# lunarlab-gatech/SLIDE_SLAM

Hardware: AMD Instinct MI355X
Metric: pose-graph updates/sec + ms/Gauss-Newton iter, 8-robot 10k-landmark graph (higher is better)
Workload: dtype f64

## Files before the change

### slide_slam_amd/csrc/chol_kernels.hip

```cpp
#include <hip/hip_runtime.h>
#include <stdlib.h>
#include <algorithm>
#include <type_traits>
#include <utility>
#include <vector>

#include "graph_dev.hpp"
#include "kernels.hpp"

namespace sl {

typedef double v4d __attribute__((ext_vector_type(4)));
constexpr int CHOL_BATCH_MAX = 8;
__device__ inline v4d mfma_f64(double a, double b, v4d c) { return __builtin_amdgcn_mfma_f64_16x16x4f64(a, b, c, 0, 0, 0); }

__device__ inline double rsqrt_nr(double d) {
#ifdef SLIDE_RSQRT_OLD
  double y = __builtin_amdgcn_rsq(d);
  y = y * (1.5 - 0.5 * d * y * y);
  y = y * (1.5 - 0.5 * d * y * y);
  return y;
#else
  double y = __builtin_amdgcn_rsq(d);
  double t = d * y, h = 0.5 * y;
// ... 1736 lines not shown
}

struct ExtractArgs { int n; const double* S[CHOL_STEP_BATCH_MAX]; int ld[CHOL_STEP_BATCH_MAX]; int T[CHOL_STEP_BATCH_MAX]; int Tr[CHOL_STEP_BATCH_MAX]; double* yv[CHOL_STEP_BATCH_MAX]; double* dp[CHOL_STEP_BATCH_MAX]; int* status[CHOL_STEP_BATCH_MAX]; };
__global__ void k_chol_extract_y_b(ExtractArgs A) {
  const int r = blockIdx.y;
  const int c = blockIdx.x * blockDim.x + threadIdx.x;
  if (c == 0) A.status[r][4] = 0;
  if (c < A.T[r] * NB) {
    A.yv[r][c] = A.S[r][(size_t)c * A.ld[r] + (size_t)A.Tr[r] * NB];
    A.dp[r][c] = __longlong_as_double((long long)BWD_SENT);
  }
}

constexpr int CHAIN_THREADS = 320;
struct alignas(16) ChainLds {
  alignas(16) double xs[2][NB];
  alignas(16) double ys[NB];
  alignas(16) double red[4][NB];
  alignas(16) double Lo[6][256];
  alignas(16) double Ws[4][256];
  alignas(16) double tmp[3][256];
  alignas(16) double Ms[NB][NB + 1];
};
template <bool F32, bool WFIRE = false>
__device__ __forceinline__ void bwd_chain_body(ChainLds& W, const double* __restrict__ S, int ld, int T, const double* __restrict__ Ld,
                                               const double* __restrict__ Winv, const double* __restrict__ yv, double* dp, int* status, int bidx,
                                               const float* __restrict__ L32, const int* __restrict__ prof,
                                               const double* __restrict__ wf_prev = nullptr, double wf_thr = 0.0, int wf_Tprev = 0,
                                               int* wf_lds = nullptr, int wf_lim = 0) {
  int dummy_state = 0;
  int& wf_state = WFIRE ? *wf_lds : dummy_state;
  auto& Ms = W.Ms; auto& Lo = W.Lo; auto& Ws = W.Ws; auto& tmp = W.tmp; auto& xs = W.xs; auto& ys = W.ys;
  const int tid = threadIdx.x;
  const bool worker = tid < 256;
  CSTAMP(0);
  const int c = T - 1 - bidx;
  if (WFIRE) {
    if (tid == 0) wf_state = 0;
    __syncthreads();
  }
  const int col = tid >> 2, part = tid & 3;
  const int jtop = prof ? prof[c] : T - 1;
  const int nj = jtop - c;
  constexpr int RB = F32 ? 6 : 3;
  typedef typename std::conditional<F32, float, double>::type tile_t;
  tile_t tr[RB][16];
  const double* tcol = S + (size_t)(c * NB + col) * ld + 16 * part;
  const float* pcol = F32 ? L32 + ((size_t)c * (T - 1) - (size_t)c * (c - 1) / 2) * (NB * NB) + col * NB + 16 * part : nullptr;
  auto tile_load = [&](tile_t (&dst)[16], int q) {
    if (F32) {
      const float4* tp = reinterpret_cast<const float4*>(pcol + (size_t)(nj - 1 - q) * (NB * NB));
#pragma unroll
// ... 4 lines not shown
    } else {
      const double* tp = tcol + (size_t)(jtop - q) * NB;
#pragma unroll
      for (int r = 0; r < 16; ++r) dst[r] = tp[r];
    }
  };
  double y0 = 0.0;
  if (worker) {
#pragma unroll
    for (int q = 0; q < RB; ++q)
      if (q < nj) tile_load(tr[q], q);
    y0 = yv[c * NB + col];
  }
  if (worker) {
    const double* Ldk = Ld + (size_t)c * NB * NB;
    const double* Wk = Winv + (size_t)c * 1024;
#pragma unroll
    for (int b = 1; b < 4; ++b)
#pragma unroll
      for (int a = 0; a < b; ++a) Lo[b * (b - 1) / 2 + a][tid] = Ldk[(size_t)(16 * a + (tid >> 4)) * NB + 16 * b + (tid & 15)];
#pragma unroll
    for (int b = 0; b < 4; ++b) Ws[b][tid] = Wk[(size_t)b * 256 + tid];
  }
  __syncthreads();
  {
    const int r = tid & 15, cc = (tid >> 4) & 15;
    if (worker) {
#pragma unroll
      for (int b = 0; b < 4; ++b) Ms[16 * b + r][16 * b + cc] = Ws[b][cc * 16 + r];
    }
    __syncthreads();
#pragma unroll
    for (int d = 1; d < 4; ++d) {
#pragma unroll
      for (int a = 0; a + d < 4; ++a) {
        const int b = a + d;
        double t = 0.0;
#pragma unroll
        for (int m = a; m < b; ++m)
#pragma unroll
          for (int n = 0; n < 16; ++n) t += Lo[b * (b - 1) / 2 + m][n * 16 + r] * Ms[16 * m + n][16 * a + cc];
        if (worker) tmp[a][cc * 16 + r] = t;
      }
      __syncthreads();
#pragma unroll
      for (int a = 0; a + d < 4; ++a) {
        const int b = a + d;
// ... 60 lines not shown
        }
      }
    }
  }
  CSTAMP(4);
  if (WFIRE && wf_state != 0) {
    if (tid < NB) __hip_atomic_store(dp + (size_t)c * NB + tid, wf_prev[(size_t)c * NB + tid], __ATOMIC_RELAXED, __HIP_MEMORY_SCOPE_AGENT);
    if (tid == 0) {
      if (wf_state == 2) atomicMax(status + 7, c);
      atomicAdd(status + 3, 1);
    }
    return;
  }
  acc += __shfl_xor(acc, 1);
  acc += __shfl_xor(acc, 2);
  if (worker && part == 0) ys[col] = y0 - acc;
  __syncthreads();
  CSTAMP(5);
  double x = 0.0;
#pragma unroll
  for (int r = 0; r < 16; ++r) x += mreg[r] * ys[16 * part + r];
  x += __shfl_xor(x, 1);
  x += __shfl_xor(x, 2);
  if (worker && part == 0) __hip_atomic_store(dp + (size_t)c * NB + col, x, __ATOMIC_RELAXED, __HIP_MEMORY_SCOPE_AGENT);
  CSTAMP(6);
}
__device__ __forceinline__ int bwd_ticket(int* ctr) {
  __shared__ int s_t;
  if (threadIdx.x == 0) s_t = atomicAdd(ctr, 1);
  __syncthreads();
  const int t = s_t;
  __syncthreads();
  return t;
}
__global__ __launch_bounds__(CHAIN_THREADS) void k_chol_bwd_chain(const double* __restrict__ S, int ld, int T, const double* __restrict__ Ld,
                                                        const double* __restrict__ Winv, const double* __restrict__ yv, double* dp, int* status,
                                                        const int* __restrict__ prof) {
  __shared__ ChainLds W;
  const int t = bwd_ticket(&status[4]);
  if (t >= T) return;
  bwd_chain_body<false>(W, S, ld, T, Ld, Winv, yv, dp, status, t, nullptr, prof);
}
__global__ __launch_bounds__(CHAIN_THREADS) void k_chol_bwd_chain_wf(const double* __restrict__ S, int ld, int T, const double* __restrict__ Ld,
                                                           const double* __restrict__ Winv, const double* __restrict__ yv, double* dp, int* status,
                                                           const int* __restrict__ prof, const double* __restrict__ prev, double thr, int Tprev, int lim) {
  __shared__ ChainLds W;
  __shared__ int s_wf;
  const int t = bwd_ticket(&status[4]);
  if (t >= T) return;
  bwd_chain_body<false, true>(W, S, ld, T, Ld, Winv, yv, dp, status, t, nullptr, prof, prev, thr, Tprev, &s_wf, lim);
}
constexpr int BWD_BATCH_MAX = 32;
struct BwdBatchArgs {
  int n;
  const double* S[BWD_BATCH_MAX]; int ld[BWD_BATCH_MAX]; int T[BWD_BATCH_MAX];
  const double* Ld[BWD_BATCH_MAX]; const double* Winv[BWD_BATCH_MAX]; const double* yv[BWD_BATCH_MAX]; double* dp[BWD_BATCH_MAX];
  int* status[BWD_BATCH_MAX];
  const int* prof[BWD_BATCH_MAX];
  int base[BWD_BATCH_MAX + 1];
  int Tmax;
};
__global__ __launch_bounds__(CHAIN_THREADS) void k_chol_bwd_chain_batched(BwdBatchArgs A) {
  __shared__ ChainLds W;
  for (;;) {
    const int t = bwd_ticket(&A.status[0][4]);
    if (t >= A.n * A.Tmax) return;
    const int r = t % A.n, b = t / A.n;
    if (b >= A.T[r]) continue;
    bwd_chain_body<false>(W, A.S[r], A.ld[r], A.T[r], A.Ld[r], A.Winv[r], A.yv[r], A.dp[r], A.status[r], b, nullptr, A.prof[r]);
    return;
  }
}


enum { TAB_MF = 0, TAB_MB = 1, TAB_PF = 2, TAB_PB = 3 };
struct ChainTabArgs {
  int n; int T[CHOL_BATCH_MAX]; const double* S[CHOL_BATCH_MAX]; int ld[CHOL_BATCH_MAX];
  const double* Ld[CHOL_BATCH_MAX]; const double* Winv[CHOL_BATCH_MAX]; const int* prof[CHOL_BATCH_MAX]; double* ctab[CHOL_BATCH_MAX];
};
__global__ __launch_bounds__(256) void k_chain_tables(ChainTabArgs A) {
  __shared__ ChainLds W;
  __shared__ double Ts[NB][NB];
  auto& Ms = W.Ms; auto& Lo = W.Lo; auto& Ws = W.Ws; auto& tmp = W.tmp;
  const int sys = blockIdx.y, c = blockIdx.x, tid = threadIdx.x;
  const int T = A.T[sys];
  if (c >= T) return;
  {
    const double* Ldk = A.Ld[sys] + (size_t)c * NB * NB;
    const double* Wk = A.Winv[sys] + (size_t)c * 1024;
#pragma unroll
    for (int b = 1; b < 4; ++b)
#pragma unroll
// ... 599 lines not shown
      acc += w[t * NB + lane] * x[t * NB + lane];
    }
  } else {
    for (int q = lane; q < nrow; q += 64) acc += w[q] * x[q];
  }
#pragma unroll
  for (int m = 32; m >= 1; m >>= 1) acc += __shfl_xor(acc, m);
  if (lane == 0) A.yv[r][col] -= acc;
}
void launch_border_apply(const CholSystem* d, int n, const double* const* xloc, hipStream_t s) {
  BorderApplyArgs A{};
  A.n = n;
  int Tmax = 0;
  for (int i = 0; i < n; ++i) {
    A.S[i] = d[i].S; A.ld[i] = d[i].ld; A.T[i] = d[i].T; A.nbr[i] = d[i].nbr; A.yv[i] = d[i].yv; A.x[i] = xloc[i];
    A.b0[i] = d[i].b0 > 0 ? d[i].b0 : d[i].T;
    A.segtab[i] = d[i].segtab;
    Tmax = d[i].T > Tmax ? d[i].T : Tmax;
  }
  if (Tmax > 0) hipLaunchKernelGGL(k_border_apply, dim3(Tmax * NB / 4, 1, n), dim3(256), 0, s, A);
}

void launch_chol_bwd_all(const double* S, int ld, int T, const double* Ld, const double* Winv, double* yv, double* dp,
                         int* status, const int* prof, hipStream_t s, const double* wf_prev, double wf_thr, int wf_Tprev, int wf_lim);
void launch_chol_extract_y(const double* S, int ld, int T, double* yv, double* dp, int* status, hipStream_t s, int nbr, int b0, double* prev) {
  hipLaunchKernelGGL(k_chol_extract_y, dim3((T * NB + 255) / 256), dim3(256), 0, s, S, ld, T, (b0 > 0 ? b0 : T) + nbr, yv, dp, status, prev);
}
struct StepPlan { int kb, nP, g0, g1, nX, TvA, TvB, TvX, nbA, nbB, nbX; long long nA, nB; };
static int chol_n_cu() {
  static int n_cu = 0;
  if (!n_cu) {
    int dev = 0;
    hipDeviceProp_t pr;
    if (hipGetDevice(&dev) == hipSuccess && hipGetDeviceProperties(&pr, dev) == hipSuccess) n_cu = pr.multiProcessorCount;
    if (n_cu <= 0) n_cu = 256;
  }
  return n_cu;
}
static StepPlan plan_step(int k, int T, const int* prof, int nbr = 0, const int* bfirst = nullptr, int kofs = 0) {
  static const double frac = getenv("SLIDE_CHOL_FRAC") ? atof(getenv("SLIDE_CHOL_FRAC")) : 0.5;
  StepPlan p{};
  p.kb = k & ~1;
  p.TvA = p.TvB = p.TvX = T;
  if (prof && k < T) {
    p.TvA = prof[k] + 1;
    if (p.kb >= 1) p.TvB = prof[p.kb - 1] + 1;
    if (k >= 1) p.TvX = prof[k - 1] + 1;
// ... 185 lines not shown
  if (!solve) {
    ExtractArgs E{};
    E.n = n;
    for (int i = 0; i < n; ++i) {
      E.S[i] = d[i].S; E.ld[i] = d[i].ld; E.T[i] = d[i].T; E.Tr[i] = (d[i].b0 > 0 ? d[i].b0 : d[i].T) + d[i].nbr;
      E.yv[i] = d[i].yv; E.dp[i] = d[i].dp; E.status[i] = d[i].status;
    }
    if (Tmax > 0) hipLaunchKernelGGL(k_chol_extract_y_b, dim3((Tmax * NB + 255) / 256, n), dim3(256), 0, s, E);
    return;
  }
  launch_chain_tables(d, n, s);
  const double* yin[CHOL_BATCH_MAX];
  double* xout[CHOL_BATCH_MAX];
  for (int i = 0; i < n; ++i) {
    launch_chol_extract_y(d[i].S, d[i].ld, d[i].T, d[i].yv, d[i].dp, d[i].status, s, d[i].nbr);
    yin[i] = d[i].yv; xout[i] = d[i].dp;
  }
  if (chain_has_tables(d, n)) {
    launch_chain_batch(d, n, yin, xout, false, false, true, nullptr, s);
    return;
  }
  launch_chol_bwd_batch(d, n, s);
}
void launch_chol_bwd_batch(const CholSystem* d, int n, hipStream_t s) {
  if (n > BWD_BATCH_MAX) {
    for (int lo = 0; lo < n; lo += BWD_BATCH_MAX) launch_chol_bwd_batch(d + lo, n - lo < BWD_BATCH_MAX ? n - lo : BWD_BATCH_MAX, s);
    return;
  }
  BwdBatchArgs B{};
  B.n = n;
  B.base[0] = 0;
  int Tmax = 0;
  for (int i = 0; i < n; ++i) {
    B.S[i] = d[i].S; B.ld[i] = d[i].ld; B.T[i] = d[i].T; B.Ld[i] = d[i].Ld; B.Winv[i] = d[i].Winv; B.yv[i] = d[i].yv; B.dp[i] = d[i].dp;
    B.status[i] = d[i].status;
    B.prof[i] = d[i].prof;
    B.base[i + 1] = B.base[i] + d[i].T;
    Tmax = d[i].T > Tmax ? d[i].T : Tmax;
  }
  B.Tmax = Tmax;
  if (B.base[n] <= 0) return;
  hipLaunchKernelGGL(k_chol_bwd_chain_batched, dim3(B.base[n]), dim3(CHAIN_THREADS), 0, s, B);
}
void launch_chol_solve_bwd(const CholSystem& cs, hipStream_t s) {
  if (chain_has_tables(&cs, 1)) {
    launch_chain_tables(&cs, 1, s);
    const double* yin = cs.yv;
    double* xout = cs.dp;
    launch_chain_batch(&cs, 1, &yin, &xout, false, false, true, nullptr, s);
    return;
  }
  launch_chol_bwd_all(cs.S, cs.ld, cs.T, cs.Ld, cs.Winv, cs.yv, cs.dp, cs.status, cs.prof, s);
}
void launch_chol_bwd_all(const double* S, int ld, int T, const double* Ld, const double* Winv, double* yv, double* dp,
                         int* status, const int* prof, hipStream_t s, const double* wf_prev, double wf_thr, int wf_Tprev, int wf_lim) {
  if (wf_lim < 0 || wf_lim > wf_Tprev) wf_lim = wf_Tprev;
  if (wf_prev && wf_thr > 0.0 && wf_Tprev > 0 && wf_lim > 0)
    hipLaunchKernelGGL(k_chol_bwd_chain_wf, dim3(T), dim3(CHAIN_THREADS), 0, s, S, ld, T, Ld, Winv, yv, dp, status, prof, wf_prev, wf_thr, wf_Tprev, wf_lim);
  else
    hipLaunchKernelGGL(k_chol_bwd_chain, dim3(T), dim3(CHAIN_THREADS), 0, s, S, ld, T, Ld, Winv, yv, dp, status, prof);
}

struct CholLLPlan {
  LLSys* d_sys = nullptr; LLTask* d_tasks = nullptr; int* d_ints = nullptr;
  int n_sys = 0, n_tasks = 0, n_ints = 0, n_chain = 0, max_cols = 0;
};
CholLLPlan* chol_ll_plan_create(const CholSystem* d, int n, const int* const* h_ord, hipStream_t up) {
  static const int ll_mode = getenv("SLIDE_LL_MODE") ? atoi(getenv("SLIDE_LL_MODE")) : 0;
  std::vector<LLSys> sys(n);
  std::vector<std::vector<int>> first(n), bf(n), bphys(n), profv(n);
  size_t n_ints = 16;
  int Tmax = 0;
  for (int i = 0; i < n; ++i) {
    const CholSystem& c = d[i];
    LLSys& y = sys[i];
    y.S = c.S; y.Ld = c.Ld; y.Winv = c.Winv; y.status = c.status; y.ld = c.ld; y.T = c.T; y.B0 = c.b0 > 0 ? c.b0 : c.T; y.nbr = c.nbr;
    y.frows = y.B0 + y.nbr + 1;
    y.flags = reinterpret_cast<int*>(n_ints);
    n_ints += (size_t)y.T * y.frows;
    Tmax = c.T > Tmax ? c.T : Tmax;
    profv[i].resize(c.T);
    for (int k = 0; k < c.T; ++k) profv[i][k] = c.h_prof ? std::min(c.h_prof[k], c.T - 1) : c.T - 1;
    first[i].assign(c.T, 0);
// ... 138 lines not shown
```

### slide_slam_amd/csrc/host_graph.hip

```cpp
#include <chrono>

#include "host_graph.hpp"

#include <algorithm>
#include <cmath>
#include <cstdio>
#include <cstdlib>
#include <map>
#include <unordered_map>

namespace sl {

static inline int lam_ks_cap(int nl) {
  const int tiles = (nl + 1) * nl;
  if (tiles <= 0) return 1;
  return tiles <= 32 ? 16 : std::max(1, std::min(16, 256 / tiles));
}

thread_local std::string g_last_error;
void thread_capture_mode_local() {
  thread_local bool done = false;
  if (done) return;
  hipStreamCaptureMode m = hipStreamCaptureModeThreadLocal;
  (void)hipThreadExchangeStreamCaptureMode(&m);
// ... 532 lines not shown
    SL_HIP(hipStreamSynchronize(master));
  }
  if (!d_pair_tickets && chol_pair_mask() != 0) {
    SL_HIP(hipMalloc(reinterpret_cast<void**>(&d_pair_tickets), 12 * CHOL_STEP_BATCH_MAX * sizeof(int)));
    SL_HIP(hipMemsetAsync(d_pair_tickets, 0, 12 * CHOL_STEP_BATCH_MAX * sizeof(int), master));
    SL_HIP(hipStreamSynchronize(master));
  }
  if (!d_Gs) SL_HIP(hipMalloc(reinterpret_cast<void**>(&d_Gs), CHOL_BATCH_HOST_MAX * sizeof(GraphDev)));
  if (!d_status_all) SL_HIP(hipMalloc(reinterpret_cast<void**>(&d_status_all), CHOL_BATCH_HOST_MAX * 8 * sizeof(int)));
  SL_HIP(hipMemcpyAsync(d_Gs, hG.data(), n * sizeof(GraphDev), hipMemcpyHostToDevice, master));
  if (rb.on()) {
    hR.resize(n);
    for (int i = 0; i < n; ++i) hR[i] = member_view(graphs[i]);
    if (!d_Rs) SL_HIP(hipMalloc(reinterpret_cast<void**>(&d_Rs), CHOL_BATCH_HOST_MAX * sizeof(RobustDev)));
    SL_HIP(hipMemcpyAsync(d_Rs, hR.data(), n * sizeof(RobustDev), hipMemcpyHostToDevice, master));
  }
  if (ol.on()) {
    hO.resize(n);
    for (int i = 0; i < n; ++i) hO[i] = member_obs_view(graphs[i]);
    if (!d_Os) SL_HIP(hipMalloc(reinterpret_cast<void**>(&d_Os), CHOL_BATCH_HOST_MAX * sizeof(ObsLossDev)));
    SL_HIP(hipMemcpyAsync(d_Os, hO.data(), n * sizeof(ObsLossDev), hipMemcpyHostToDevice, master));
  }
  SL_HIP(hipStreamSynchronize(master));
  seg_sys.clear(); l2_sys.clear(); l2_graph.clear(); seg_hord.clear();
  free_ll_band_plans();
  if (arrow && hG[0].n_slots > 0) {
    for (int i = 0; i < n; ++i) {
      HostGraph* g = graphs[i];
      const GraphDev& G = hG[i];
      if (G.nsep <= 0 || g->segs.empty()) { seg_sys.push_back(sys[i]); seg_hord.push_back(nullptr); continue; }
      for (size_t k = 0; k < g->segs.size(); ++k) {
        const HostGraph::Seg sg = g->segs[k];
        CholSystem c = sys[i];
        c.S = G.S + (size_t)sg.t0 * NB * G.ld + (size_t)sg.t0 * NB;
        c.T = sg.t1 - sg.t0;
        c.Ld = G.Ld + (size_t)sg.t0 * NB * NB; c.Winv = G.Winv + (size_t)sg.t0 * 1024;
        c.yv = G.yv + (size_t)sg.t0 * NB; c.dp = G.dp + (size_t)sg.t0 * NB;
        c.h_prof = g->seg_prof[k].data(); c.prof = g->d_seg_prof.d + g->seg_prof_off[k]; c.first = nullptr;
        c.b0 = G.T - sg.t0; c.kofs = sg.t0;
        c.L32 = nullptr; c.ctab = nullptr;
        const int* hord = nullptr;
        if (k < g->seg_ord.size() && !getenv("SLIDE_SEG_PLAIN")) {
          c.h_bfirst = g->seg_sfirst[k].data();
          c.ord = g->d_seg_ord.d + k * (size_t)G.nbr;
          hord = g->seg_ord[k].data();
        }
        seg_sys.push_back(c);
        seg_hord.push_back(hord);
      }
      if (!g->seg_tab.empty() && !getenv("SLIDE_SEG_PLAIN")) sys[i].segtab = g->d_seg_tab.d;
      CholSystem l2{};
      l2.S = G.bord; l2.ld = G.ldb; l2.T = G.nsep; l2.Ld = g->d_Ld2.d; l2.Winv = g->d_Winv2.d; l2.yv = g->d_yv2.d; l2.dp = g->d_dp2.d;
      l2.status = G.status; l2.nbr = G.nbr - G.nsep;
      l2.bord = G.bord + (size_t)G.nsep * NB * G.ldb + (size_t)G.nsep * NB; l2.ldb = G.ldb;
      l2_sys.push_back(l2);
      l2_graph.push_back(i);
    }
    {
      std::vector<std::pair<int, int>> jl;
      for (int i = 0; i < n; ++i) {
        const int nb = sys[i].nbr, T = sys[i].T;
        const int* hb = sys[i].h_bfirst;
        if (nb > 1023 || n > 2047) { jl.clear(); break; }
        const std::vector<int>& stb = graphs[i]->seg_tab;
        const bool seg = sys[i].segtab != nullptr && !stb.empty();
        for (int jb = 0; jb < nb; ++jb)
          for (int ib = jb; ib <= nb; ++ib) {
            int K = T - (hb ? std::max(hb[ib], hb[jb]) : 0);
            if (seg) {
              K = 0;
              const int NS = stb[0];
// ... 492 lines not shown
      if (e1) (void)hipEventRecord(e1, master);
    } else {
      const int rc = factor_all(e1);
      if (rc != SLIDE_OK) return rc;
    }
    mark(1);
    if (n_syrk_jobs > 0) launch_border_syrk_jobs(sys.data(), n, d_syrk_jobs, n_syrk_jobs, syrk_lds_pad, master);
    else launch_border_syrk(sys.data(), n, master);
    mark(6);
    if (!l2_sys.empty()) {
      if (ll_l2) launch_chol_ll(ll_l2, l2_sys.data(), (int)l2_sys.size(), master);
      else launch_chol_batch(l2_sys.data(), (int)l2_sys.size(), d_ctr2, master, nullptr, false, 100, (chol_pair_mask() & 2) ? pair_tickets(8) : nullptr);
      if (n_l2_jobs > 0) launch_border_syrk_jobs(l2_sys.data(), (int)l2_sys.size(), d_l2_jobs, n_l2_jobs, 0, master);
      else launch_border_syrk(l2_sys.data(), (int)l2_sys.size(), master);
    }
    mark(2);
    static const bool env_canon = !(getenv("SLIDE_SEP_CANONICAL") && getenv("SLIDE_SEP_CANONICAL")[0] == '0');
    const bool canon = whole && sep_dissected() && env_canon && n <= 8;
    if (canon) launch_sep_gather(hG.data(), n, maps, Y, false, master, d_sep_tmask, sTL * NB, sep_mask_b, sep_top2, sep_ld2, sep_bord2);
    else launch_sep_gather(hG.data(), n, maps, Y, !whole, master, d_sep_tmask);
    mark(3);
  }
  if (whole || part == 2) {
    if (!whole && !owned) launch_sep_unpack(Y, master);
    if (owned) launch_sep_unpack(Y, master, sTL, sep_Ts + sep_nl);
    if (sep_dissected()) {
      const int TL = sTL, Tt = sTt;
      static const bool env_canon2 = !(getenv("SLIDE_SEP_CANONICAL") && getenv("SLIDE_SEP_CANONICAL")[0] == '0');
      const bool canon2 = whole && env_canon2 && n <= 8;
      if (!owned) {
        if (ll_leaves) launch_chol_ll(ll_leaves, lv, 2, master);
        else launch_chol_batch(lv, 2, sep_ctr2, master, nullptr, false, 100, (chol_pair_mask() & 4) ? pair_tickets(9) : nullptr);
        if (canon2) {
          CholSystem tp2[2] = {top, top};
          for (int hh = 0; hh < 2; ++hh) {
            tp2[hh].S = sepS + (size_t)(hh ? sTa : 0) * NB * ld_s; tp2[hh].T = sep_leafT[hh]; tp2[hh].b0 = sTL;
            if (hh) { tp2[hh].bord = sep_top2; tp2[hh].ldb = sep_ld2; }
          }
          CholSystem sl2[2];
          int ks_lam[2] = {1, 1};
          for (int hh = 0; hh < 2 && sep_nl > 0; ++hh) {
            CholSystem sl{};
            sl.S = sepS + (size_t)(hh ? sTa : 0) * NB * ld_s; sl.ld = ld_s; sl.T = sep_leafT[hh]; sl.b0 = sep_Ts; sl.nbr = sep_nl;
            sl.bord = hh ? sep_bord2 : sep_bord; sl.ldb = (sep_nl + 1) * NB;
            ks_lam[hh] = std::max(1, std::min(lam_ks_cap(sep_nl), sep_leafT[hh] / 2));
            sl2[hh] = sl;
// ... 31 lines not shown
      const CholSystem ts = sep_top_system();
      launch_chol_batch(&ts, 1, sep_ctr, master, nullptr, false, 100, pair_tickets(11));
    } else {
      for (int k = 0; k < sep_Ts; ++k)
        launch_chol_step(sepS, ld_s, k, sep_Ts, sep_Ld + (size_t)k * NB * NB, sep_Winv + (size_t)k * 1024, sep_status, sep_ctr, nullptr,
                         sep_prof_on ? h_sep_prof.data() : nullptr, master, sep_nl);
      launch_chol_extract_y(sepS, ld_s, sep_Ts, sep_yv, sep_dp, sep_status, master, sep_nl);
    }
    if (sep_nl > 0) {
      CholSystem ss{};
      ss.S = sepS; ss.ld = ld_s; ss.T = sep_Ts; ss.yv = sep_yv; ss.nbr = sep_nl; ss.bord = sep_bord; ss.ldb = (sep_nl + 1) * NB; ss.bfirst = nullptr;
      CholSystem sr = ss;
      static const bool env_canon3 = !(getenv("SLIDE_SEP_CANONICAL") && getenv("SLIDE_SEP_CANONICAL")[0] == '0');
      if (owned || (whole && sep_dissected() && env_canon3 && n <= 8)) { sr.S = sepS + (size_t)sTL * NB * ld_s; sr.T = sTt; sr.b0 = sep_Ts; }
      const int ks = std::max(1, std::min(lam_ks_cap(sep_nl), sr.T / 2));
      launch_border_syrk(&sr, 1, master, lam_scratch, ks);
      launch_lam_prepare(sep_bord, sep_nl, sep_lam, lamS, master);
      const int ld_l = (sep_nl + 1) * NB;
      for (int k = 0; k < sep_nl; ++k)
        launch_chol_step(lamS, ld_l, k, sep_nl, lam_Ld + (size_t)k * NB * NB, lam_Winv + (size_t)k * 1024, lam_status, lam_ctr, nullptr, nullptr, master);
      launch_chol_extract_y(lamS, ld_l, sep_nl, lam_yv, lam_dp, lam_status, master);
      launch_chol_bwd_all(lamS, ld_l, sep_nl, lam_Ld, lam_Winv, lam_yv, lam_dp, lam_status, nullptr, master);
      const double* xl = lam_dp;
      if (!owned) launch_border_apply(&ss, 1, &xl, master);
      else {
        CholSystem ap2[2] = {ss, ss};
        ap2[0].S = sepS + (size_t)own_t0 * NB * ld_s; ap2[0].T = own_T; ap2[0].b0 = sep_Ts; ap2[0].yv = sep_yv + (size_t)own_t0 * NB;
        ap2[1].S = sepS + (size_t)sTL * NB * ld_s; ap2[1].T = sTt; ap2[1].b0 = sep_Ts; ap2[1].yv = sep_yv + (size_t)sTL * NB;
        const double* xl2[2] = {xl, xl};
        launch_border_apply(ap2, 2, xl2, master);
      }
    }
    if (sep_dissected()) {
      double* St = sepS + (size_t)sTL * NB * ld_s + (size_t)sTL * NB;
      launch_chol_bwd_all(St, ld_s, sTt, sep_Ld + (size_t)sTL * NB * NB, sep_Winv + (size_t)sTL * 1024, sep_yv + (size_t)sTL * NB, sep_dp + (size_t)sTL * NB,
                          sep_status, nullptr, master);
      launch_ints_clear(sep_status + 4, 1, master);
      CholSystem ap[2] = {lv[0], lv[1]};
      ap[0].nbr = ap[1].nbr = sTt;
      const double* xt[2] = {sep_dp + (size_t)sTL * NB, sep_dp + (size_t)sTL * NB};
      if (!owned) {
        launch_border_apply(ap, 2, xt, master);
        launch_chol_bwd_batch(lv, 2, master);
      } else {
        launch_border_apply(&ap[own], 1, xt, master);
        launch_chol_bwd_batch(&lv[own], 1, master);
      }
    } else {
      launch_chol_bwd_all(sepS, ld_s, sep_Ts, sep_Ld, sep_Winv, sep_yv, sep_dp, sep_status, sep_prof_on ? d_sep_prof : nullptr, master);
    }
    mark(4);
    launch_sep_xloc(n, maps, sep_m, sep_lam, sep_dp, lam_dp, xloc, master);
    if (!l2_sys.empty()) {
      const double* x2[CHOL_BATCH_HOST_MAX];
      for (size_t i = 0; i < l2_sys.size(); ++i) x2[i] = xloc[l2_graph[i]] + (size_t)hG[l2_graph[i]].nsep * NB;
      launch_border_apply(l2_sys.data(), (int)l2_sys.size(), x2, master);
      launch_chol_bwd_batch(l2_sys.data(), (int)l2_sys.size(), master);
      launch_ints_clear(l2_sys[0].status + 4, 1, master);
      {
        const double* src[CHOL_BATCH_HOST_MAX]; double* dst[CHOL_BATCH_HOST_MAX]; int cnt[CHOL_BATCH_HOST_MAX];
        for (size_t i = 0; i < l2_sys.size(); ++i) { src[i] = l2_sys[i].dp; dst[i] = xloc[l2_graph[i]]; cnt[i] = hG[l2_graph[i]].nsep * NB; }
        launch_copy_pairs(src, dst, cnt, (int)l2_sys.size(), master);
      }
    }
    launch_border_apply(sys.data(), n, xloc, master);
    launch_chol_bwd_batch(seg_sys.data(), (int)seg_sys.size(), master);
    launch_sep_pose_scatter_batched(d_Gs, hG.data(), n, xloc, master);
    bool slots_onto = true;
    for (int i = 0; i < n; ++i) slots_onto = slots_onto && graphs[i]->lm_slot_onto;
    launch_arrow_finish_batched(d_Gs, hG.data(), n, sep_dp, d_sep_off, master, slots_onto);
    launch_status_gather(d_Gs, n, d_status_all, master, sep_status, sep_nl > 0 ? lam_status : nullptr);
    mark(5);
  }
  return SLIDE_OK;
}
int CholBatch::profile_arrow(double* const* d_bufs, double* out6, int* n_sep_steps) {
  std::lock_guard<std::mutex> pl(pass_mtx);
  exact_serial = 0;
  bool same = false;
  int rc = begin_pass(d_bufs, &same);
  if (rc != SLIDE_OK) return rc;
  if (!(arrow && hG[0].n_slots > 0)) { g_last_error = "profile_arrow: the batch does not run exact joint passes"; return SLIDE_ERR_INVALID; }
  hipEvent_t start = nullptr;
  SL_HIP(hipEventCreate(&start));
  for (auto& e : prof_ev) SL_HIP(hipEventCreate(&e));
  (void)hipEventRecord(start, master);
  rc = enqueue_arrow(d_bufs, -1, nullptr, nullptr);
  const hipError_t es = hipStreamSynchronize(master);
  if (rc == SLIDE_OK && es == hipSuccess) {
// ... 1631 lines not shown
```

### slide_slam_amd/csrc/host_graph.hpp

```cpp
#pragma once
#include <hip/hip_runtime.h>

#include <cstdint>
#include <cstring>
#include <condition_variable>
#include <functional>
#include <mutex>
#include <string>
#include <unordered_map>
#include <vector>

#include "../../include/slide_gpu.h"
#include "graph_dev.hpp"
#include "kernels.hpp"
#include "sl_math.hpp"

namespace sl {

extern thread_local std::string g_last_error;
void thread_capture_mode_local();
bool hip_ok(hipError_t e, const char* what);
inline bool robot_ok(int r) { return r >= 0 && r < SLIDE_MAX_ROBOTS; }
int decode_status(const int* st8);
struct LossSetting {
// ... 171 lines not shown

 private:
  int n;
  std::mutex mtx;
  std::mutex pass_mtx;
  bool pass_dirty = false;
  std::condition_variable cv;
  int arrived = 0;
  unsigned long long generation = 0;
  int gen_status = SLIDE_OK;
  std::vector<CholSystem> sys;
  std::vector<double*> bufs;
  std::vector<HostGraph*> graphs;
  hipGraphExec_t pass_exec = nullptr;
  hipGraphExec_t part_exec[7] = {nullptr, nullptr, nullptr, nullptr, nullptr, nullptr, nullptr};
  int enqueue_ghost_refresh(double* const* d_bufs, int part);
  int last_part = -1;
  int pcg_iters = 0;
  double pcg_tol = 0.0;
  bool arrow = false;
  int n_seg = 1;
  std::vector<CholSystem> seg_sys, l2_sys;
  std::vector<int> l2_graph;
  int* d_ctr2 = nullptr;
  int* d_pair_tickets = nullptr;
  int* pair_tickets(int block) const { return d_pair_tickets ? d_pair_tickets + block * CHOL_STEP_BATCH_MAX : nullptr; }
  CholLLPlan *ll_seg = nullptr, *ll_l2 = nullptr, *ll_leaves = nullptr, *ll_leaf_own[2] = {nullptr, nullptr}, *ll_top = nullptr;
  std::vector<const int*> seg_hord;
  void free_ll_band_plans();
  void free_ll_sep_plans();
  void sep_leaf_systems(CholSystem* lv) const;
  CholSystem sep_top_system() const;
  int* d_syrk_jobs = nullptr;
  int n_syrk_jobs = 0, syrk_jobs_cap = 0, syrk_lds_pad = 0;
  int* d_l2_jobs = nullptr; int n_l2_jobs = 0, l2_jobs_cap = 0;
  double* sepS = nullptr; long long sep_len = 0;
  double* sep_x = nullptr; long long sep_x_len = 0;
  int sep_m = 0, sep_Ts = 0;
  double *sep_Ld = nullptr, *sep_Winv = nullptr, *sep_yv = nullptr, *sep_dp = nullptr;
  int *sep_status = nullptr, *sep_ctr = nullptr, *d_sep_off = nullptr;
  int sep_cap = 0;
  std::vector<int> h_sep_prof; int* d_sep_prof = nullptr; bool sep_prof_on = false;
  int sep_leafT[2] = {0, 0}, sep_used[2] = {0, 0};
  int sep_owner = -1; bool sep_leader = true;
  std::vector<int> h_leaf_prof[2];
  int* d_leaf_prof = nullptr;
// ... 358 lines not shown
```

### slide_slam_amd/csrc/kernels.hpp

```cpp
#pragma once
#include <hip/hip_runtime.h>
#include <stdint.h>

#include "graph_dev.hpp"
#include "sl_math.hpp"

namespace sl {

void init_solver_kernels();
void launch_relin(const GraphDev& G, hipStream_t s);
void launch_linearize(const GraphDev& G, const ObsLossDev& O, hipStream_t s);
void launch_observation_weights(const GraphDev& G, const ObsLossDev& O, bool robust, int n, double* out2n, hipStream_t s);
void launch_observation_weights_batched(const GraphDev* d, const ObsLossDev* dO, bool robust, const int* off, const int* cnt, int n, double* out2n,
                                        hipStream_t s);
void launch_robust_reweight(const GraphDev& G, const RobustDev& R, hipStream_t s);
void launch_closure_weights(const GraphDev& G, const RobustDev& R, const int* idx, int n, double* out2n, hipStream_t s);
void launch_robust_reweight_batched(const GraphDev* d, const RobustDev* dR, const GraphDev* h, int n, hipStream_t s);
void launch_closure_weights_batched(const GraphDev* d, const RobustDev* dR, const int* ent2, int n, double* out2n, hipStream_t s);
void launch_landmark(const GraphDev& G, int mode, hipStream_t s);
void launch_pose(const GraphDev& G, hipStream_t s);
void launch_schur(const GraphDev& G, hipStream_t s);
void launch_backsub(const GraphDev& G, int mode, hipStream_t s);
void launch_shared_pack(const GraphDev& G, int what, double* buf, hipStream_t s);
void launch_shared_unpack(const GraphDev& G, int what, const double* buf, hipStream_t s);
// ... 32 lines not shown
AsmMerge asm_merge_env();
void launch_phase3_arrow_batched(const GraphDev* d, const GraphDev* h, int n, hipStream_t s);

void launch_chol_step(double* S, int ld, int k, int T, double* Ld, double* Winv, int* status, int* ctr, float* L32, const int* h_prof, hipStream_t s, int nbr = 0);
void launch_chol_extract_y(const double* S, int ld, int T, double* yv, double* dp, int* status, hipStream_t s, int nbr = 0, int b0 = 0, double* prev = nullptr);
constexpr unsigned long long CHAIN_SENTINEL = 0x7FF8DEADBEEF0BADull;
struct CholSystem { double* S; int ld, T; double* Ld; double* Winv; double* yv; double* dp; int* status;
                    float* L32;
                    const int* h_prof;
                    const int* prof; const int* first;
                    double* ctab;
                    int nbr;
                    double* bord; int ldb;
                    const double* bord_src;
                    const int* bfirst;
                    const int* h_bfirst;
                    int b0;
                    int kofs;
                    const int* ord;
                    const int* segtab; };
constexpr int CHOL_STEP_BATCH_MAX = 32;
void launch_chol_batch(const CholSystem* d, int n, int* ctr, hipStream_t s, hipEvent_t after_steps = nullptr, bool solve = true, int cu_share = 100, int* pair_tickets = nullptr);
bool chol_pair_supported(const CholSystem* d, int n);
void launch_chol_bwd_batch(const CholSystem* d, int n, hipStream_t s);
struct CholLLPlan;
CholLLPlan* chol_ll_plan_create(const CholSystem* d, int n, const int* const* h_ord = nullptr, hipStream_t upload_stream = nullptr);
void chol_ll_plan_destroy(CholLLPlan* p);
int chol_ll_plan_tasks(const CholLLPlan* p);
int chol_ll_plan_columns(const CholLLPlan* p);
void launch_chol_ll(const CholLLPlan* p, const CholSystem* d, int n, hipStream_t s, int* trace = nullptr);
void launch_border_syrk(const CholSystem* d, int n, hipStream_t s, double* scratch = nullptr, int ks = 1);
void launch_border_syrk_jobs(const CholSystem* d, int n, const int* jobs, int njobs, int lds_pad, hipStream_t s, double* scratch = nullptr, int ks = 1, int jb_end = -1,
                             const int* ks_sys = nullptr, bool fuse_add = false);
void launch_border_apply(const CholSystem* d, int n, const double* const* xloc, hipStream_t s);
void launch_chain_batch(const CholSystem* d, int n, const double* const* in, double* const* out, bool fwd, bool f32, bool prepared,
                        double* const* next_out, hipStream_t s);
void launch_chain_tables(const CholSystem* d, int n, hipStream_t s);
void launch_chol_bwd_all(const double* S, int ld, int T, const double* Ld, const double* Winv, double* yv, double* dp, int* status, const int* prof, hipStream_t s,
                         const double* wf_prev = nullptr, double wf_thr = 0.0, int wf_Tprev = 0, int wf_lim = -1);
void launch_pose_covariance(const double* S, int ld, int T, const double* Ld, const double* Winv, double* Y, int row0, double* cov36,
                            hipStream_t s);
void launch_selected_inverse(const double* S, int ld, int T, const double* Ld, const double* Winv, const int* prof, const int* d_prof,
                             double* Sg, double* Z, hipStream_t s);
void launch_pose_blocks(const double* Sg, int ld, const int* poses, int n, double* out, hipStream_t s, const int* prow = nullptr);
void launch_landmark_covariances(const GraphDev& G, const double* Sg, int ld, const int* lids, int n, double* out, hipStream_t s,
                                 const int* prow = nullptr);
void launch_multi_solve(const double* S, int ld, int T, const double* Ld, const double* Winv, const int* prof, double* B, double* X,
                        int nrhs, hipStream_t s);
void launch_multi_fwd(const double* S, int ld, int T, const double* Ld, const double* Winv, const int* prof, double* B, double* W,
                      int nrhs, hipStream_t s);
void launch_gram(const double* X, size_t ldx, int ncol, const int* rows, int nrows, double* M, hipStream_t s);
void launch_landmark_V(const GraphDev& G, const double* U, int nT, int ncol, const int* lids, int n, double* V, size_t ldv, hipStream_t s,
                       const int* prow = nullptr);
void launch_scatter(const int* rc, const double* val, int n, double* B, int nT, hipStream_t s);
constexpr int GAIN_MAX_STEPS = 64, GAIN_MAX_GRAMS = 4, GAIN_LDS_DIM = 96;
struct GainCandDev { int c0, nk, nsplit, pad; long long moff, poff, woff; };
int gain_gram_splits(int nk);
void launch_gram_blocks(const double* X, size_t ldx, const int* rows, int nrows, const GainCandDev* cand, int ncand, const int4* jobs,
                        int njobs, double* part, double* M, hipStream_t s);
int launch_woodbury_blocks(const double* U, size_t ldu, const GainCandDev* cand, int ncand, const int* jptr, const int* jrow,
                           const double* jval, const double* M, size_t msz, int nM, double* work, double* gains, int* flag, bool small,
                           bool big, hipStream_t s);
// ... 190 lines not shown
```

Before: 3997.

## Fuse border-apply into backward chain solve and self-reset ticket counters

Folds the border matrix-vector correction (formerly separate launch_border_apply kernels) into the backward chain kernel prologue, where each block computes its own border contribution, with an optional segment-mask skip. It also lets the last ticket holder reset the ticket counter, which removes separate clear launches, and writes results directly into xloc to drop a copy kernel. The default mask of 6 enables ticket reset and the direct write, while border fusion stays behind bit 1 and is off by default. The trade-off is extra per-block work and reduced-parallelism border loads inside the serial chain.

```diff
diff --git a/slide_slam_amd/csrc/chol_kernels.hip b/slide_slam_amd/csrc/chol_kernels.hip
--- a/slide_slam_amd/csrc/chol_kernels.hip
+++ b/slide_slam_amd/csrc/chol_kernels.hip
@@ -1782,12 +1782,49 @@
   alignas(16) double tmp[3][256];
   alignas(16) double Ms[NB][NB + 1];
 };
+__device__ __forceinline__ void chain_border_term(double* __restrict__ out, const double* __restrict__ S, int ld, int c, const double* __restrict__ xb,
+                                                  const int* __restrict__ st, int b0, int nbr, int kofs, int tid) {
+  const int wv = tid >> 6, lane = tid & 63;
+  const double* w = S + (size_t)(c * NB + 16 * wv) * ld + (size_t)b0 * NB + lane;
+  const double* x = xb + lane;
+  double a[16];
+#pragma unroll
+  for (int k = 0; k < 16; ++k) a[k] = 0.0;
+  const int* msk = st ? st + 1 + st[0] + st[0] * (nbr + 1) : nullptr;
+  if (msk && msk[0] > 0) {
+    const int cb = c + kofs;
+    unsigned long long m = (unsigned long long)(unsigned)msk[1 + 2 * cb] | ((unsigned long long)(unsigned)msk[2 + 2 * cb] << 32);
+    while (m) {
+      const int t = __ffsll((long long)m) - 1;
+      m &= m - 1;
+      const double xv = x[t * NB];
+#pragma unroll
+      for (int k = 0; k < 16; ++k) a[k] += w[(size_t)k * ld + t * NB] * xv;
+    }
+  } else {
+    for (int t = 0; t < nbr; ++t) {
+      const double xv = x[t * NB];
+#pragma unroll
+      for (int k = 0; k < 16; ++k) a[k] += w[(size_t)k * ld + t * NB] * xv;
+    }
+  }
+#pragma unroll
+  for (int k = 0; k < 16; ++k) {
+#pragma unroll
+    for (int m = 32; m >= 1; m >>= 1) a[k] += __shfl_xor(a[k], m);
+  }
+  if (lane == 0) {
+#pragma unroll
+    for (int k = 0; k < 16; ++k) out[16 * wv + k] = a[k];
+  }
+}
 template <bool F32, bool WFIRE = false>
 __device__ __forceinline__ void bwd_chain_body(ChainLds& W, const double* __restrict__ S, int ld, int T, const double* __restrict__ Ld,
                                                const double* __restrict__ Winv, const double* __restrict__ yv, double* dp, int* status, int bidx,
                                                const float* __restrict__ L32, const int* __restrict__ prof,
                                                const double* __restrict__ wf_prev = nullptr, double wf_thr = 0.0, int wf_Tprev = 0,
-                                               int* wf_lds = nullptr, int wf_lim = 0) {
+                                               int* wf_lds = nullptr, int wf_lim = 0,
+                                               const ChainBorder bx0 = ChainBorder{}, const ChainBorder bx1 = ChainBorder{}, double* __restrict__ dp2 = nullptr) {
   int dummy_state = 0;
   int& wf_state = WFIRE ? *wf_lds : dummy_state;
   auto& Ms = W.Ms; auto& Lo = W.Lo; auto& Ws = W.Ws; auto& tmp = W.tmp; auto& xs = W.xs; auto& ys = W.ys;
@@ -1838,7 +1875,16 @@
 #pragma unroll
     for (int b = 0; b < 4; ++b) Ws[b][tid] = Wk[(size_t)b * 256 + tid];
   }
+  const bool has_b0 = bx0.x != nullptr && bx0.nbr > 0, has_b1 = bx1.x != nullptr && bx1.nbr > 0;
+  if (worker) {
+    if (has_b0) chain_border_term(W.red[0], S, ld, c, bx0.x, bx0.segtab, bx0.b0, bx0.nbr, bx0.kofs, tid);
+    if (has_b1) chain_border_term(W.red[1], S, ld, c, bx1.x, bx1.segtab, bx1.b0, bx1.nbr, bx1.kofs, tid);
+  }
   __syncthreads();
+  if (worker) {
+    if (has_b0) y0 = y0 - W.red[0][col];
+    if (has_b1) y0 = y0 - W.red[1][col];
+  }
   {
     const int r = tid & 15, cc = (tid >> 4) & 15;
     if (worker) {
@@ -1945,12 +1991,19 @@
   for (int r = 0; r < 16; ++r) x += mreg[r] * ys[16 * part + r];
   x += __shfl_xor(x, 1);
   x += __shfl_xor(x, 2);
-  if (worker && part == 0) __hip_atomic_store(dp + (size_t)c * NB + col, x, __ATOMIC_RELAXED, __HIP_MEMORY_SCOPE_AGENT);
+  if (worker && part == 0) {
+    __hip_atomic_store(dp + (size_t)c * NB + col, x, __ATOMIC_RELAXED, __HIP_MEMORY_SCOPE_AGENT);
+    if (dp2) dp2[(size_t)c * NB + col] = x;
+  }
   CSTAMP(6);
 }
-__device__ __forceinline__ int bwd_ticket(int* ctr) {
+__device__ __forceinline__ int bwd_ticket(int* ctr, int last = -1) {
   __shared__ int s_t;
-  if (threadIdx.x == 0) s_t = atomicAdd(ctr, 1);
+  if (threadIdx.x == 0) {
+    const int t = atomicAdd(ctr, 1);
+    if (t == last) __hip_atomic_store(ctr, 0, __ATOMIC_RELAXED, __HIP_MEMORY_SCOPE_AGENT);
+    s_t = t;
+  }
   __syncthreads();
   const int t = s_t;
   __syncthreads();
@@ -1958,18 +2011,19 @@
 }
 __global__ __launch_bounds__(CHAIN_THREADS) void k_chol_bwd_chain(const double* __restrict__ S, int ld, int T, const double* __restrict__ Ld,
                                                         const double* __restrict__ Winv, const double* __restrict__ yv, double* dp, int* status,
-                                                        const int* __restrict__ prof) {
+                                                        const int* __restrict__ prof, ChainExtra X, int last) {
   __shared__ ChainLds W;
-  const int t = bwd_ticket(&status[4]);
+  const int t = bwd_ticket(&status[4], last);
   if (t >= T) return;
-  bwd_chain_body<false>(W, S, ld, T, Ld, Winv, yv, dp, status, t, nullptr, prof);
+  bwd_chain_body<false>(W, S, ld, T, Ld, Winv, yv, dp, status, t, nullptr, prof, nullptr, 0.0, 0, nullptr, 0, X.b[0], X.b[1], X.dp2);
 }
 __global__ __launch_bounds__(CHAIN_THREADS) void k_chol_bwd_chain_wf(const double* __restrict__ S, int ld, int T, const double* __restrict__ Ld,
                                                            const double* __restrict__ Winv, const double* __restrict__ yv, double* dp, int* status,
-                                                           const int* __restrict__ prof, const double* __restrict__ prev, double thr, int Tprev, int lim) {
+                                                           const int* __restrict__ prof, const double* __restrict__ prev, double thr, int Tprev, int lim,
+                                                           int last) {
   __shared__ ChainLds W;
   __shared__ int s_wf;
-  const int t = bwd_ticket(&status[4]);
+  const int t = bwd_ticket(&status[4], last);
   if (t >= T) return;
   bwd_chain_body<false, true>(W, S, ld, T, Ld, Winv, yv, dp, status, t, nullptr, prof, prev, thr, Tprev, &s_wf, lim);
 }
@@ -1982,15 +2036,21 @@
   const int* prof[BWD_BATCH_MAX];
   int base[BWD_BATCH_MAX + 1];
   int Tmax;
+  int last;
+  const double* x0[BWD_BATCH_MAX]; const int* st0[BWD_BATCH_MAX]; int b00[BWD_BATCH_MAX]; int nbr0[BWD_BATCH_MAX]; int kofs0[BWD_BATCH_MAX];
+  const double* x1[BWD_BATCH_MAX]; int b01[BWD_BATCH_MAX]; int nbr1[BWD_BATCH_MAX];
+  double* dp2[BWD_BATCH_MAX];
 };
+static_assert(sizeof(BwdBatchArgs) <= 4096, "kernel arguments: at most 4 KB");
 __global__ __launch_bounds__(CHAIN_THREADS) void k_chol_bwd_chain_batched(BwdBatchArgs A) {
   __shared__ ChainLds W;
   for (;;) {
-    const int t = bwd_ticket(&A.status[0][4]);
+    const int t = bwd_ticket(&A.status[0][4], A.last);
     if (t >= A.n * A.Tmax) return;
     const int r = t % A.n, b = t / A.n;
     if (b >= A.T[r]) continue;
-    bwd_chain_body<false>(W, A.S[r], A.ld[r], A.T[r], A.Ld[r], A.Winv[r], A.yv[r], A.dp[r], A.status[r], b, nullptr, A.prof[r]);
+    bwd_chain_body<false>(W, A.S[r], A.ld[r], A.T[r], A.Ld[r], A.Winv[r], A.yv[r], A.dp[r], A.status[r], b, nullptr, A.prof[r], nullptr, 0.0, 0, nullptr, 0,
+                          ChainBorder{A.x0[r], A.st0[r], A.b00[r], A.nbr0[r], A.kofs0[r]}, ChainBorder{A.x1[r], nullptr, A.b01[r], A.nbr1[r], 0}, A.dp2[r]);
     return;
   }
 }
@@ -2636,7 +2696,8 @@
 }
 
 void launch_chol_bwd_all(const double* S, int ld, int T, const double* Ld, const double* Winv, double* yv, double* dp,
-                         int* status, const int* prof, hipStream_t s, const double* wf_prev, double wf_thr, int wf_Tprev, int wf_lim);
+                         int* status, const int* prof, hipStream_t s, const double* wf_prev, double wf_thr, int wf_Tprev, int wf_lim,
+                         const ChainExtra* ex, bool reset_ticket);
 void launch_chol_extract_y(const double* S, int ld, int T, double* yv, double* dp, int* status, hipStream_t s, int nbr, int b0, double* prev) {
   hipLaunchKernelGGL(k_chol_extract_y, dim3((T * NB + 255) / 256), dim3(256), 0, s, S, ld, T, (b0 > 0 ? b0 : T) + nbr, yv, dp, status, prev);
 }
@@ -2868,21 +2929,35 @@
   }
   launch_chol_bwd_batch(d, n, s);
 }
-void launch_chol_bwd_batch(const CholSystem* d, int n, hipStream_t s) {
+BackMerge back_merge_env() {
+  BackMerge M{6};
+  if (const char* e = getenv("SLIDE_BACK_MERGE")) M.mask = atoi(e);
+  return M;
+}
+void launch_chol_bwd_batch(const CholSystem* d, int n, hipStream_t s, const ChainExtra* ex, bool reset_ticket) {
   if (n > BWD_BATCH_MAX) {
-    for (int lo = 0; lo < n; lo += BWD_BATCH_MAX) launch_chol_bwd_batch(d + lo, n - lo < BWD_BATCH_MAX ? n - lo : BWD_BATCH_MAX, s);
+    for (int lo = 0; lo < n; lo += BWD_BATCH_MAX)
+      launch_chol_bwd_batch(d + lo, n - lo < BWD_BATCH_MAX ? n - lo : BWD_BATCH_MAX, s, ex ? ex + lo : nullptr, reset_ticket);
     return;
   }
   BwdBatchArgs B{};
   B.n = n;
   B.base[0] = 0;
   int Tmax = 0;
+  B.last = -1;
   for (int i = 0; i < n; ++i) {
     B.S[i] = d[i].S; B.ld[i] = d[i].ld; B.T[i] = d[i].T; B.Ld[i] = d[i].Ld; B.Winv[i] = d[i].Winv; B.yv[i] = d[i].yv; B.dp[i] = d[i].dp;
     B.status[i] = d[i].status;
     B.prof[i] = d[i].prof;
     B.base[i + 1] = B.base[i] + d[i].T;
     Tmax = d[i].T > Tmax ? d[i].T : Tmax;
+    if (reset_ticket && d[i].T > 0) B.last = std::max(B.last, i + n * (d[i].T - 1));
+    if (ex) {
+      const ChainBorder &b0 = ex[i].b[0], &b1 = ex[i].b[1];
+      B.x0[i] = b0.x; B.st0[i] = b0.segtab; B.b00[i] = b0.b0; B.nbr0[i] = b0.nbr; B.kofs0[i] = b0.kofs;
+      B.x1[i] = b1.x; B.b01[i] = b1.b0; B.nbr1[i] = b1.nbr;
+      B.dp2[i] = ex[i].dp2;
+    }
   }
   B.Tmax = Tmax;
   if (B.base[n] <= 0) return;
@@ -2899,12 +2974,14 @@
   launch_chol_bwd_all(cs.S, cs.ld, cs.T, cs.Ld, cs.Winv, cs.yv, cs.dp, cs.status, cs.prof, s);
 }
 void launch_chol_bwd_all(const double* S, int ld, int T, const double* Ld, const double* Winv, double* yv, double* dp,
-                         int* status, const int* prof, hipStream_t s, const double* wf_prev, double wf_thr, int wf_Tprev, int wf_lim) {
+                         int* status, const int* prof, hipStream_t s, const double* wf_prev, double wf_thr, int wf_Tprev, int wf_lim,
+                         const ChainExtra* ex, bool reset_ticket) {
   if (wf_lim < 0 || wf_lim > wf_Tprev) wf_lim = wf_Tprev;
+  const int last = reset_ticket ? T - 1 : -1;
   if (wf_prev && wf_thr > 0.0 && wf_Tprev > 0 && wf_lim > 0)
-    hipLaunchKernelGGL(k_chol_bwd_chain_wf, dim3(T), dim3(CHAIN_THREADS), 0, s, S, ld, T, Ld, Winv, yv, dp, status, prof, wf_prev, wf_thr, wf_Tprev, wf_lim);
+    hipLaunchKernelGGL(k_chol_bwd_chain_wf, dim3(T), dim3(CHAIN_THREADS), 0, s, S, ld, T, Ld, Winv, yv, dp, status, prof, wf_prev, wf_thr, wf_Tprev, wf_lim, last);
   else
-    hipLaunchKernelGGL(k_chol_bwd_chain, dim3(T), dim3(CHAIN_THREADS), 0, s, S, ld, T, Ld, Winv, yv, dp, status, prof);
+    hipLaunchKernelGGL(k_chol_bwd_chain, dim3(T), dim3(CHAIN_THREADS), 0, s, S, ld, T, Ld, Winv, yv, dp, status, prof, ex ? *ex : ChainExtra{}, last);
 }
 
 struct CholLLPlan {
diff --git a/slide_slam_amd/csrc/host_graph.hip b/slide_slam_amd/csrc/host_graph.hip
--- a/slide_slam_amd/csrc/host_graph.hip
+++ b/slide_slam_amd/csrc/host_graph.hip
@@ -578,13 +578,13 @@
     SL_HIP(hipMemcpyAsync(d_Os, hO.data(), n * sizeof(ObsLossDev), hipMemcpyHostToDevice, master));
   }
   SL_HIP(hipStreamSynchronize(master));
-  seg_sys.clear(); l2_sys.clear(); l2_graph.clear(); seg_hord.clear();
+  seg_sys.clear(); l2_sys.clear(); l2_graph.clear(); seg_hord.clear(); seg_graph.clear();
   free_ll_band_plans();
   if (arrow && hG[0].n_slots > 0) {
     for (int i = 0; i < n; ++i) {
       HostGraph* g = graphs[i];
       const GraphDev& G = hG[i];
-      if (G.nsep <= 0 || g->segs.empty()) { seg_sys.push_back(sys[i]); seg_hord.push_back(nullptr); continue; }
+      if (G.nsep <= 0 || g->segs.empty()) { seg_sys.push_back(sys[i]); seg_hord.push_back(nullptr); seg_graph.push_back(i); continue; }
       for (size_t k = 0; k < g->segs.size(); ++k) {
         const HostGraph::Seg sg = g->segs[k];
         CholSystem c = sys[i];
@@ -603,6 +603,7 @@
         }
         seg_sys.push_back(c);
         seg_hord.push_back(hord);
+        seg_graph.push_back(i);
       }
       if (!g->seg_tab.empty() && !getenv("SLIDE_SEG_PLAIN")) sys[i].segtab = g->d_seg_tab.d;
       CholSystem l2{};
@@ -1141,6 +1142,7 @@
     mark(3);
   }
   if (whole || part == 2) {
+    const int back = back_merge_env().mask;
     if (!whole && !owned) launch_sep_unpack(Y, master);
     if (owned) launch_sep_unpack(Y, master, sTL, sep_Ts + sep_nl);
     if (sep_dissected()) {
@@ -1218,7 +1220,8 @@
       launch_chol_extract_y(lamS, ld_l, sep_nl, lam_yv, lam_dp, lam_status, master);
       launch_chol_bwd_all(lamS, ld_l, sep_nl, lam_Ld, lam_Winv, lam_yv, lam_dp, lam_status, nullptr, master);
       const double* xl = lam_dp;
-      if (!owned) launch_border_apply(&ss, 1, &xl, master);
+      if (back & 1) {
+      } else if (!owned) launch_border_apply(&ss, 1, &xl, master);
       else {
         CholSystem ap2[2] = {ss, ss};
         ap2[0].S = sepS + (size_t)own_t0 * NB * ld_s; ap2[0].T = own_T; ap2[0].b0 = sep_Ts; ap2[0].yv = sep_yv + (size_t)own_t0 * NB;
@@ -1227,40 +1230,67 @@
         launch_border_apply(ap2, 2, xl2, master);
       }
     }
+    auto lam_term = [&](int t0) { return ((back & 1) && sep_nl > 0) ? ChainBorder{lam_dp, nullptr, sep_Ts - t0, sep_nl, 0} : ChainBorder{}; };
     if (sep_dissected()) {
       double* St = sepS + (size_t)sTL * NB * ld_s + (size_t)sTL * NB;
+      ChainExtra et{};
+      et.b[0] = lam_term(sTL);
       launch_chol_bwd_all(St, ld_s, sTt, sep_Ld + (size_t)sTL * NB * NB, sep_Winv + (size_t)sTL * 1024, sep_yv + (size_t)sTL * NB, sep_dp + (size_t)sTL * NB,
-                          sep_status, nullptr, master);
-      launch_ints_clear(sep_status + 4, 1, master);
+                          sep_status, nullptr, master, nullptr, 0.0, 0, -1, &et, (back & 2) != 0);
+      if (!(back & 2)) launch_ints_clear(sep_status + 4, 1, master);
       CholSystem ap[2] = {lv[0], lv[1]};
       ap[0].nbr = ap[1].nbr = sTt;
       const double* xt[2] = {sep_dp + (size_t)sTL * NB, sep_dp + (size_t)sTL * NB};
+      ChainExtra el[2] = {};
+      if (back & 1)
+        for (int b = 0; b < 2; ++b) {
+          el[b].b[0] = lam_term(b ? sTa : 0);
+          el[b].b[1] = ChainBorder{xt[b], nullptr, lv[b].b0, sTt, 0};
+        }
       if (!owned) {
-        launch_border_apply(ap, 2, xt, master);
-        launch_chol_bwd_batch(lv, 2, master);
+        if (!(back & 1)) launch_border_apply(ap, 2, xt, master);
+        launch_chol_bwd_batch(lv, 2, master, el);
       } else {
-        launch_border_apply(&ap[own], 1, xt, master);
-        launch_chol_bwd_batch(&lv[own], 1, master);
+        if (!(back & 1)) launch_border_apply(&ap[own], 1, xt, master);
+        launch_chol_bwd_batch(&lv[own], 1, master, &el[own]);
       }
     } else {
-      launch_chol_bwd_all(sepS, ld_s, sep_Ts, sep_Ld, sep_Winv, sep_yv, sep_dp, sep_status, sep_prof_on ? d_sep_prof : nullptr, master);
+      ChainExtra et{};
+      et.b[0] = lam_term(0);
+      launch_chol_bwd_all(sepS, ld_s, sep_Ts, sep_Ld, sep_Winv, sep_yv, sep_dp, sep_status, sep_prof_on ? d_sep_prof : nullptr, master, nullptr, 0.0, 0, -1, &et);
     }
     mark(4);
     launch_sep_xloc(n, maps, sep_m, sep_lam, sep_dp, lam_dp, xloc, master);
     if (!l2_sys.empty()) {
       const double* x2[CHOL_BATCH_HOST_MAX];
-      for (size_t i = 0; i < l2_sys.size(); ++i) x2[i] = xloc[l2_graph[i]] + (size_t)hG[l2_graph[i]].nsep * NB;
-      launch_border_apply(l2_sys.data(), (int)l2_sys.size(), x2, master);
-      launch_chol_bwd_batch(l2_sys.data(), (int)l2_sys.size(), master);
-      launch_ints_clear(l2_sys[0].status + 4, 1, master);
-      {
+      ChainExtra e2[CHOL_BATCH_HOST_MAX] = {};
+      for (size_t i = 0; i < l2_sys.size(); ++i) {
+        x2[i] = xloc[l2_graph[i]] + (size_t)hG[l2_graph[i]].nsep * NB;
+        if (back & 1) e2[i].b[0] = ChainBorder{x2[i], nullptr, l2_sys[i].T, l2_sys[i].nbr, 0};
+        if (back & 4) e2[i].dp2 = xloc[l2_graph[i]];
+      }
+      if (!(back & 1)) launch_border_apply(l2_sys.data(), (int)l2_sys.size(), x2, master);
+      launch_chol_bwd_batch(l2_sys.data(), (int)l2_sys.size(), master, e2, (back & 2) != 0);
+      if (!(back & 2)) launch_ints_clear(l2_sys[0].status + 4, 1, master);
+      if (!(back & 4)) {
         const double* src[CHOL_BATCH_HOST_MAX]; double* dst[CHOL_BATCH_HOST_MAX]; int cnt[CHOL_BATCH_HOST_MAX];
         for (size_t i = 0; i < l2_sys.size(); ++i) { src[i] = l2_sys[i].dp; dst[i] = xloc[l2_graph[i]]; cnt[i] = hG[l2_graph[i]].nsep * NB; }
         launch_copy_pairs(src, dst, cnt, (int)l2_sys.size(), master);
       }
     }
-    launch_border_apply(sys.data(), n, xloc, master);
-    launch_chol_bwd_batch(seg_sys.data(), (int)seg_sys.size(), master);
+    if (back & 1) {
+      std::vector<ChainExtra> es(seg_sys.size());
+      for (size_t i = 0; i < seg_sys.size(); ++i) {
+        const CholSystem& c = seg_sys[i];
+        const int g = seg_graph[i];
+        es[i] = ChainExtra{};
+        es[i].b[0] = ChainBorder{xloc[g], sys[g].segtab, c.b0 > 0 ? c.b0 : c.T, sys[g].nbr, c.kofs};
+      }
+      launch_chol_bwd_batch(seg_sys.data(), (int)seg_sys.size(), master, es.data());
+    } else {
+      launch_border_apply(sys.data(), n, xloc, master);
+      launch_chol_bwd_batch(seg_sys.data(), (int)seg_sys.size(), master);
+    }
     launch_sep_pose_scatter_batched(d_Gs, hG.data(), n, xloc, master);
     bool slots_onto = true;
     for (int i = 0; i < n; ++i) slots_onto = slots_onto && graphs[i]->lm_slot_onto;
diff --git a/slide_slam_amd/csrc/host_graph.hpp b/slide_slam_amd/csrc/host_graph.hpp
--- a/slide_slam_amd/csrc/host_graph.hpp
+++ b/slide_slam_amd/csrc/host_graph.hpp
@@ -217,6 +217,7 @@
   int n_seg = 1;
   std::vector<CholSystem> seg_sys, l2_sys;
   std::vector<int> l2_graph;
+  std::vector<int> seg_graph;
   int* d_ctr2 = nullptr;
   int* d_pair_tickets = nullptr;
   int* pair_tickets(int block) const { return d_pair_tickets ? d_pair_tickets + block * CHOL_STEP_BATCH_MAX : nullptr; }
diff --git a/slide_slam_amd/csrc/kernels.hpp b/slide_slam_amd/csrc/kernels.hpp
--- a/slide_slam_amd/csrc/kernels.hpp
+++ b/slide_slam_amd/csrc/kernels.hpp
@@ -78,7 +78,11 @@
 constexpr int CHOL_STEP_BATCH_MAX = 32;
 void launch_chol_batch(const CholSystem* d, int n, int* ctr, hipStream_t s, hipEvent_t after_steps = nullptr, bool solve = true, int cu_share = 100, int* pair_tickets = nullptr);
 bool chol_pair_supported(const CholSystem* d, int n);
-void launch_chol_bwd_batch(const CholSystem* d, int n, hipStream_t s);
+struct BackMerge { int mask; };
+BackMerge back_merge_env();
+struct ChainBorder { const double* x; const int* segtab; int b0, nbr, kofs; };
+struct ChainExtra { ChainBorder b[2]; double* dp2; };
+void launch_chol_bwd_batch(const CholSystem* d, int n, hipStream_t s, const ChainExtra* ex = nullptr, bool reset_ticket = false);
 struct CholLLPlan;
 CholLLPlan* chol_ll_plan_create(const CholSystem* d, int n, const int* const* h_ord = nullptr, hipStream_t upload_stream = nullptr);
 void chol_ll_plan_destroy(CholLLPlan* p);
@@ -93,7 +97,8 @@
                         double* const* next_out, hipStream_t s);
 void launch_chain_tables(const CholSystem* d, int n, hipStream_t s);
 void launch_chol_bwd_all(const double* S, int ld, int T, const double* Ld, const double* Winv, double* yv, double* dp, int* status, const int* prof, hipStream_t s,
-                         const double* wf_prev = nullptr, double wf_thr = 0.0, int wf_Tprev = 0, int wf_lim = -1);
+                         const double* wf_prev = nullptr, double wf_thr = 0.0, int wf_Tprev = 0, int wf_lim = -1,
+                         const ChainExtra* ex = nullptr, bool reset_ticket = false);
 void launch_pose_covariance(const double* S, int ld, int T, const double* Ld, const double* Winv, double* Y, int row0, double* cov36,
                             hipStream_t s);
 void launch_selected_inverse(const double* S, int ld, int T, const double* Ld, const double* Winv, const int* prof, const int* d_prof,
```

Result: no change. 4008, median of 3 (+0.3%).
